# naggender2/distributed-lms-raft-llm

Hardware: AMD Instinct MI355X
Metric: tutoring tokens/sec (GPT-2-124M) + p50 query latency at 1/2/4/8 MI355X (higher is better)
Workload: dtype bf16; 1 GPU; model=gpt2 (124M), global_batch=1024, seq_len=150, prompt_len=32, decode=greedy + repetition_penalty 1.2, max_length 150 (tutoring_server.py:21-29), parallelism=dp1, hipgraph=True, device=AMD Radeon Graphics

## Files before the change

### distributed_lms_raft_llm_amd/ops/__init__.py

```python
from __future__ import annotations

import ctypes
import os
import subprocess
import threading
from pathlib import Path

import torch

_HERE = Path(__file__).resolve().parent
CSRC = _HERE / "csrc"
LIB_DIR = _HERE / "_lib"
LIB_PATH = LIB_DIR / "libdlms_hip.so"
CHECKED_LIB_PATH = LIB_DIR / "libdlms_hip_checked.so"
CHECK_UNITS = ("gemm", "attention", "decode", "encoder", "skinny", "gemm_ps", "sample")
CHECK_SITES = {1: "embed token id", 2: "position id", 3: "decode_update slot_map", 4: "decode_update token id",
               5: "decode_update sequence length", 6: "seen_set row", 7: "QKV scatter slot", 8: "QKV scatter position",
               9: "attention slot", 10: "BERT token id", 11: "seen_set token id", 12: "sampler slot_map",
               13: "sampled token id"}
SOURCES = ["api.hip", "gemm.hip", "norm.hip", "attention.hip", "decode.hip", "encoder.hip", "xgmi.hip", "skinny.hip", "gemm_ps.hip",
           "dataflow.hip", "mid.hip", "sample.hip"]
ARCH = os.environ.get("DLMS_OFFLOAD_ARCH", "gfx950")

EPI_BF16, EPI_GELU_TANH, EPI_GELU_ERF, EPI_F32, EPI_QKV, EPI_ARGMAX, EPI_PARTIAL = range(7)
# ... 1028 lines not shown

def fix_copies() -> int:
    return int(lib().dlms_fix_copies())


def fix_to_float(r: torch.Tensor) -> torch.Tensor:
    return (r.sum(0).to(torch.float64) / FIX_SCALE).to(torch.float32)


SKINNY_MLP_WIDTHS = (768, 1024, 1280, 1600)


def skinny_mlp_cg(K: int, M: int, want: int = 0) -> int:
    return int(lib().dlms_skinny_mlp_cg(K, M, want))


def skinny_mlp(x_in: torch.Tensor, gamma, beta, eps: float, w_fc_sh: torch.Tensor, b_fc, w_p_sl: torch.Tensor, b_p,
               r_out: torch.Tensor, *, parts=None, nsplit: int = 0, res_bias=None, cg: int = 0, base: bool = True):
    xfix = x_in.dtype == torch.int64
    C = fix_copies()
    xcs = 0
    if xfix:
        _req(x_in, torch.int64, "x_in", 3)
        if x_in.shape[0] != C or x_in.stride(0) % 2:
            raise ValueError(f"skinny_mlp: fixed-point x_in must be [{C}, M, d]")
        xcs = x_in.stride(0)
        x_in = x_in[0]
    else:
        _req(x_in, torch.float32, "x_in", 2)
    _req(r_out, torch.int64, "r_out", 3)
    if r_out.shape[0] != C or r_out.stride(0) % 2:
        raise ValueError(f"skinny_mlp: r_out must be [{C}, M, d]")
    rcs = r_out.stride(0)
    r_full, r_out = r_out, r_out[0]
    _req(w_fc_sh, torch.bfloat16, "w_fc_sh", 4)
    _req(w_p_sl, torch.bfloat16, "w_p_sl", 3)
    M, K = x_in.shape
    F = w_fc_sh.shape[0] * 16
    if w_fc_sh.shape[1] * 32 != K or not w_fc_sh.is_contiguous() or tuple(w_p_sl.shape) != (F // 16, K, 16) or \
            not w_p_sl.is_contiguous():
        raise ValueError("skinny_mlp: weight layouts (shuffle_weight / slice_cproj) do not match x_in")
    if M < 1 or M > 8 or K not in SKINNY_MLP_WIDTHS:
        raise ValueError(f"skinny_mlp: M <= 8 rows of width {SKINNY_MLP_WIDTHS}, got {tuple(x_in.shape)}")
    if skinny_mlp_cg(K, M, cg) == 0:
        raise ValueError(f"skinny_mlp: {M} rows of width {K} do not fit the kernel's LDS")
    if r_out.shape[0] < M or r_out.shape[1] < K or r_out.stride(1) != 1 or r_out.data_ptr() == x_in.data_ptr():
        raise ValueError("skinny_mlp: r_out too small or aliases x_in")
    if x_in.stride(1) != 1 or x_in.stride(0) % 4 or x_in.data_ptr() % 16:
        raise ValueError("skinny_mlp: x rows must be 16-byte aligned")
    for t, n, size in ((gamma, "gamma", K), (beta, "beta", K), (b_fc, "b_fc", F), (b_p, "b_p", K)):
        _req(t, torch.float32, n, 1)
        if t.numel() != size:
            raise ValueError(f"skinny_mlp: {n} size")
    if nsplit not in (0, 1, 4) or (nsplit == 4 and K > 1024):
        raise ValueError("skinny_mlp: nsplit in {0, 1, 4} (4: d <= 1024)")
    ldp, sstride = 0, 0
    if nsplit:
        _req(parts, torch.float32, "parts", 3)
        if parts.shape[0] < nsplit or parts.shape[1] < M or parts.shape[2] < K or parts.stride(2) != 1 or \
                parts.stride(1) % 4 or parts.stride(0) % 4:
            raise ValueError("skinny_mlp: parts too small / misaligned")
        ldp, sstride = parts.stride(1), parts.stride(0)
    if res_bias is not None:
        _req(res_bias, torch.float32, "res_bias", 1)
        if res_bias.numel() != K:
            raise ValueError("res_bias size")
    _check(lib().dlms_skinny_mlp(_p(x_in), x_in.stride(0), int(xfix), xcs, _p(parts) if nsplit else None, ldp,
                                 sstride, nsplit, _p(res_bias), _p(gamma), _p(beta), float(eps), _p(w_fc_sh), _p(b_fc),
                                 _p(w_p_sl), _p(b_p), _p(r_out), r_out.stride(0), rcs, M, K, F, int(cg), int(bool(base)),
                                 _stream()),
           "dlms_skinny_mlp")
    return r_full


def ln_fix(x: torch.Tensor, gamma, beta, eps: float, out: torch.Tensor):
    _req(x, torch.int64, "x", 3)
    _req(out, torch.bfloat16, "out", 2)
    if x.shape[0] != fix_copies() or x.stride(0) % 2:
        raise ValueError(f"ln_fix: x must be [{fix_copies()}, M, K]")
    xcs, x = x.stride(0), x[0]
    M, K = x.shape
    if x.stride(1) != 1 or out.stride(1) != 1 or out.shape[0] < M or out.shape[1] < K or x.stride(0) % 2 or \
            out.stride(0) % 4 or K % 4 or K > 2048 or x.data_ptr() % 16 or out.data_ptr() % 8:
        raise ValueError("ln_fix: shapes / alignment")
    for t, n in ((gamma, "gamma"), (beta, "beta")):
        _req(t, torch.float32, n, 1)
        if t.numel() != K:
            raise ValueError(f"ln_fix: {n} size")
    _check(lib().dlms_ln_fix(_p(x), x.stride(0), xcs, _p(gamma), _p(beta), float(eps), _p(out), out.stride(0), M, K,
                             _stream()), "dlms_ln_fix")
    return out


def attention_split_waves(kv_len_max: int) -> int:
    for nw in (2, 4, 8, 16):
        if kv_len_max <= 32 * nw:
            return nw
    return 16


ATTN_WS_STRIDE = 68
ATTN_SPLIT_SYNC = 2


def attention_split_geometry(pairs: int, kv_len_max: int, cus: int = 256) -> tuple[int, int]:
    nw = attention_split_waves(kv_len_max)
    if pairs <= 32 and kv_len_max > 512:
        return 8, 4
    return nw, 1


class AttnSplitWorkspace:

    def __init__(self, pairs: int, splits: int, device):
        self.pairs, self.splits = pairs, splits
        self.partials = torch.empty(pairs * splits * ATTN_WS_STRIDE, dtype=torch.float32, device=device)
        self.counters = torch.zeros(pairs, dtype=torch.int32, device=device)

    def fits(self, pairs: int, splits: int) -> bool:
        return pairs <= self.pairs and pairs * splits <= self.pairs * self.splits


def attention_split(q: torch.Tensor, k_cache: torch.Tensor, v_cache: torch.Tensor, row_slot: torch.Tensor,
                    row_kvlen: torch.Tensor, out: torch.Tensor | None = None, scale: float | None = None,
                    waves: int = 16, splits: int = 1, workspace: "AttnSplitWorkspace | None" = None,
                    sync: int | None = None):
    _req(q, torch.bfloat16, "q", 2)
    kv8 = _kv_caches(k_cache, v_cache, "attention_split")
    _req(row_slot, torch.int32, "row_slot", 1)
    _req(row_kvlen, torch.int32, "row_kvlen", 1)
    R = q.shape[0]
    S, H, T, hd = k_cache.shape
    if hd != 64 or v_cache.shape != k_cache.shape or q.shape[1] < H * 64:
        raise ValueError("attention_split: bad shapes")
    if row_slot.numel() < R or row_kvlen.numel() < R:
        raise ValueError("attention_split: index arrays too short")
    if waves not in (2, 4, 8, 16):
        raise ValueError("attention_split: waves in {2, 4, 8, 16}")
    if not 1 <= splits <= 64:
        raise ValueError("attention_split: splits in [1, 64]")
    if out is None:
        out = torch.empty(R, H * 64, dtype=torch.bfloat16, device=q.device)
    _req(out, torch.bfloat16, "out", 2)
    ws_p = cnt_p = None
    if splits > 1:
        if workspace is None:
            workspace = AttnSplitWorkspace(R * H, splits, q.device)
        if not workspace.fits(R * H, splits):
            raise ValueError("attention_split: workspace too small")
        ws_p, cnt_p = _p(workspace.partials), _p(workspace.counters)
    sc = (1.0 / 8.0) if scale is None else scale
    fn = lib().dlms_attention_split_fp8 if kv8 else lib().dlms_attention_split
    _check(fn(_p(q), q.stride(0), _p(k_cache), _p(v_cache), _p(row_slot), _p(row_kvlen), _p(out), out.stride(0), R, H, T,
              S, float(sc), int(waves), int(splits), ws_p, cnt_p, ATTN_SPLIT_SYNC if sync is None else int(sync),
              _stream()), "attention_split")
    return out


def attention_oproj_tiles(n_out: int, target_wgs: int = 16) -> int:
    G = n_out // 16
    cands = [nt for nt in (2, 3, 4, 5, 6, 8) if G % nt == 0]
    if not cands:
        raise ValueError(f"attention_oproj: N/16 = {G} has no tile count in (2,3,4,5,6,8)")
    return min(cands, key=lambda nt: (abs(G // nt - target_wgs), nt))


def attention_oproj(q: torch.Tensor, k_cache: torch.Tensor, v_cache: torch.Tensor, row_slot: torch.Tensor,
                    row_kvlen: torch.Tensor, wo_sh: torch.Tensor, parts: torch.Tensor, scale: float | None = None,
                    tiles: int | None = None) -> torch.Tensor:
    _req(q, torch.bfloat16, "q", 2)
    kv8 = _kv_caches(k_cache, v_cache, "attention_oproj")
    _req(row_slot, torch.int32, "row_slot", 1)
    _req(row_kvlen, torch.int32, "row_kvlen", 1)
    _req(wo_sh, torch.bfloat16, "wo_sh", 4)
    _req(parts, torch.float32, "parts", 3)
    M = q.shape[0]
    S, H, T, hd = k_cache.shape
    N = wo_sh.shape[0] * 16
    if not 1 <= M <= 4:
        raise ValueError("attention_oproj: 1..4 rows")
    if hd != 64 or v_cache.shape != k_cache.shape or q.shape[1] < H * 64 or wo_sh.shape[1] * 32 != H * 64:
        raise ValueError("attention_oproj: bad shapes")
    if parts.shape[0] < H or parts.shape[1] < M or parts.shape[2] < N or parts.stride(2) != 1:
        raise ValueError("attention_oproj: parts must be [>= H, >= M, >= N]")
    if row_slot.numel() < M or row_kvlen.numel() < M:
        raise ValueError("attention_oproj: index arrays too short")
    nt = attention_oproj_tiles(N) if tiles is None else tiles
    sc = (1.0 / 8.0) if scale is None else scale
    fn = lib().dlms_attention_oproj_fp8 if kv8 else lib().dlms_attention_oproj
    _check(fn(_p(q), q.stride(0), _p(k_cache), _p(v_cache), _p(row_slot), _p(row_kvlen), M, H, T, S, float(sc),
              _p(wo_sh), N, int(nt), _p(parts), parts.stride(1), parts.stride(0), _stream()),
           "attention_oproj")
    return parts


def attention_oproj_grouped(q: torch.Tensor, k_cache: torch.Tensor, v_cache: torch.Tensor, row_slot: torch.Tensor,
                            row_kvlen: torch.Tensor, wo_sh: torch.Tensor, parts: torch.Tensor, heads_per_group: int,
                            scale: float | None = None, tiles: int = 3) -> torch.Tensor:
    _req(q, torch.bfloat16, "q", 2)
    kv8 = _kv_caches(k_cache, v_cache, "attention_oproj_grouped")
    _req(row_slot, torch.int32, "row_slot", 1)
    _req(row_kvlen, torch.int32, "row_kvlen", 1)
    _req(wo_sh, torch.bfloat16, "wo_sh", 4)
    _req(parts, torch.float32, "parts", 3)
    S, H, T, hd = k_cache.shape
    N = wo_sh.shape[0] * 16
    hg = int(heads_per_group)
    if q.shape[0] != 1:
        raise ValueError("attention_oproj_grouped: one row")
    if hd != 64 or v_cache.shape != k_cache.shape or q.shape[1] < H * 64 or wo_sh.shape[1] * 32 != H * 64:
        raise ValueError("attention_oproj_grouped: bad shapes")
    if hg not in (3, 4) or H % hg or (N // 16) % tiles or tiles not in (1, 2, 3, 4):
        raise ValueError("attention_oproj_grouped: heads_per_group in {3, 4} dividing H, tiles in 1..4 dividing N/16")
    if parts.shape[0] < H // hg or parts.shape[2] < N or parts.stride(2) != 1:
        raise ValueError("attention_oproj_grouped: parts must be [>= H/hg, >= 1, >= N]")
    sc = (1.0 / 8.0) if scale is None else scale
    fn = lib().dlms_attention_oproj_grouped_fp8 if kv8 else lib().dlms_attention_oproj_grouped
    _check(fn(_p(q), _p(k_cache), _p(v_cache), _p(row_slot), _p(row_kvlen), H, hg, T, S, float(sc), _p(wo_sh), N,
              int(tiles), _p(parts), parts.stride(0), _stream()),
           "attention_oproj_grouped")
    return parts


PS_WAVES = 8


PS_LDS_BYTES = 160 * 1024


def gemm_ps_geometry(M: int, N: int, epi: int, split: int = 1, cus: int = 256, K: int = 768):
    kc = K // max(1, split)
    fits4 = 64 * (kc * 2 + 32) + 8 * 4096 <= PS_LDS_BYTES
    mt = 4 if ((epi == EPI_ARGMAX or M >= 512) and fits4) else 2
    nt = 2
    row_blocks = -(-M // (16 * mt))
    tiles = N // (16 * nt)
    need = -(-tiles // PS_WAVES)
    per_row = max(1, cus // max(1, row_blocks * split))
    col_wgs = min(need, per_row) if epi == EPI_ARGMAX else need
    return mt, nt, max(1, col_wgs)


def gemm_ps(a: torch.Tensor, w_sh: torch.Tensor, epi: int, *, bias=None, out=None, q_out=None, k_cache=None,
            v_cache=None, row_slot=None, row_pos=None, argmax_out=None, seen=None, vocab: int = 0,
            col_offset: int = 0, penalty: float = 1.0, split_k: int = 1, geometry=None):
    _req(a, torch.bfloat16, "a", 2)
    _req(w_sh, torch.bfloat16, "w_sh", 4)
    if w_sh.shape[2] != 64 or w_sh.shape[3] != 8 or not w_sh.is_contiguous():
        raise ValueError("gemm_ps: w_sh must be a contiguous shuffle_weight() tensor")
    N, K = w_sh.shape[0] * 16, w_sh.shape[1] * 32
    M = a.shape[0]
    if a.shape[1] != K or a.stride(0) % 8 or a.data_ptr() % 16:
        raise ValueError(f"gemm_ps: a {tuple(a.shape)} vs K={K} (16-byte aligned rows)")
    if split_k < 1 or K % split_k or (K // split_k) % 128:
        raise ValueError("gemm_ps: K / split_k must be a multiple of 128")
    if epi != EPI_PARTIAL and split_k != 1:
        raise ValueError("gemm_ps: split_k only with EPI_PARTIAL")
    mt, nt, col_wgs = geometry or gemm_ps_geometry(M, N, epi, split_k, K=K)
    if N % (16 * nt):
        raise ValueError("gemm_ps: N must be a multiple of 16 * nt")
    ep = GemmEpi()
    if bias is not None:
        _req(bias, torch.float32, "bias", 1)
        if bias.numel() < N:
            raise ValueError("bias too short")
        ep.bias = bias.data_ptr()
    if epi in (EPI_BF16, EPI_GELU_TANH):
        if out is None:
            out = torch.empty(M, N, dtype=torch.bfloat16, device=a.device)
        _req(out, torch.bfloat16, "out", 2)
        if out.shape[0] < M or out.shape[1] < N or out.stride(0) % 8 or out.data_ptr() % 16:
            raise ValueError("gemm_ps: out too small / misaligned")
        ep.out, ep.ldo = out.data_ptr(), out.stride(0)
    elif epi == EPI_PARTIAL:
        if out is None:
            out = torch.empty(split_k, M, N, dtype=torch.float32, device=a.device)
        _req(out, torch.float32, "out", 3)
        if out.shape[0] < split_k or out.shape[1] < M or out.shape[2] < N or out.stride(1) % 4 or \
                out.stride(0) % 4 or out.data_ptr() % 16:
            raise ValueError("gemm_ps: partial out too small / misaligned")
        ep.out, ep.ldo, ep.split_k, ep.split_stride = out.data_ptr(), out.stride(1), split_k, out.stride(0)
    elif epi == EPI_QKV:
        for t, n in ((q_out, "q_out"), (k_cache, "k_cache"), (v_cache, "v_cache")):
            _req(t, torch.bfloat16, n)
        _req(row_slot, torch.int32, "row_slot", 1)
        _req(row_pos, torch.int32, "row_pos", 1)
        if N % 3 or (N // 3) % 64:
            raise ValueError("QKV N must be 3 * d_local (64-wide heads)")
        d_local = N // 3
        if k_cache.dim() != 4 or k_cache.shape != v_cache.shape or k_cache.shape[1] * 64 != d_local or \
                k_cache.shape[3] != 64 or not k_cache.is_contiguous() or not v_cache.is_contiguous():
            raise ValueError(f"cache shape {tuple(k_cache.shape)} incompatible with d_local={d_local}")
        if q_out.shape[0] < M or q_out.shape[1] < d_local or row_slot.numel() < M or row_pos.numel() < M or \
                q_out.stride(0) % 8 or q_out.data_ptr() % 16:
            raise ValueError("qkv epilogue buffers too small / misaligned")
        ep.q_out, ep.ldq = q_out.data_ptr(), q_out.stride(0)
        ep.k_cache, ep.v_cache = k_cache.data_ptr(), v_cache.data_ptr()
        ep.row_slot, ep.row_pos = row_slot.data_ptr(), row_pos.data_ptr()
        ep.n_heads, ep.t_max, ep.d_local, ep.n_slots = k_cache.shape[1], k_cache.shape[2], d_local, k_cache.shape[0]
        out = q_out
    elif epi == EPI_ARGMAX:
        _req(argmax_out, torch.int64, "argmax_out", 2)
        _req(seen, torch.int32, "seen", 2)
        slots = PS_WAVES * col_wgs
        if argmax_out.shape[0] < M or argmax_out.shape[1] < slots or seen.shape[0] < M or \
                seen.shape[1] * 32 < vocab or col_offset % 64:
            raise ValueError("gemm_ps argmax buffers too small / misaligned shard")
        ep.argmax_out, ep.ldo, ep.seen = argmax_out.data_ptr(), argmax_out.stride(0), seen.data_ptr()
        ep.seen_words, ep.vocab, ep.col_offset, ep.penalty = seen.stride(0), vocab, col_offset, penalty
        out = argmax_out
    else:
        raise ValueError(f"gemm_ps: unsupported epilogue {epi}")
    _check(lib().dlms_gemm_ps(epi, _p(a), a.stride(0), _p(w_sh), M, N, K, split_k, mt, nt, col_wgs, ctypes.byref(ep),
                              _stream()), "dlms_gemm_ps")
    return out


def gemm_ps_key_slots(M: int, N: int, K: int = 768) -> int:
    return PS_WAVES * gemm_ps_geometry(M, N, EPI_ARGMAX, K=K)[2]
```

### distributed_lms_raft_llm_amd/ops/csrc/decode.hip

```cpp
#include "common.h"

__global__ __launch_bounds__(256) void embed_kernel(const int* __restrict__ tokens, const int* __restrict__ positions,
                                                    const bf16_t* __restrict__ wte, const bf16_t* __restrict__ wpe,
                                                    float* x, int ldx, int R, int D, int V, int P) {
    const int lane = threadIdx.x & 63;
    const int r = blockIdx.x * 4 + (threadIdx.x >> 6);
    if (r >= R) return;
    const bf16_t* a = wte + (size_t)dlms_idx(tokens[r], V, CHK_EMBED_TOKEN) * D;
    const bf16_t* b = wpe + (size_t)dlms_idx(positions[r], P, CHK_EMBED_POS) * D;
    float* o = x + (size_t)r * ldx;
    for (int c = lane; c < D / 8; c += 64) {
        float fa[8], fb[8];
        unpack8(*reinterpret_cast<const uint4*>(a + c * 8), fa);
        unpack8(*reinterpret_cast<const uint4*>(b + c * 8), fb);
        float4 lo = make_float4(fa[0] + fb[0], fa[1] + fb[1], fa[2] + fb[2], fa[3] + fb[3]);
        float4 hi = make_float4(fa[4] + fb[4], fa[5] + fb[5], fa[6] + fb[6], fa[7] + fb[7]);
        reinterpret_cast<float4*>(o + c * 8)[0] = lo;
        reinterpret_cast<float4*>(o + c * 8)[1] = hi;
    }
}

#define KEY_ROUND 16
__device__ __forceinline__ void key_round_load(const unsigned long long* __restrict__ keys, int b, int nparts,
                                               long long sb, long long sp, int lane, int p0,
                                               unsigned long long (&k)[KEY_ROUND]) {
#pragma unroll
    for (int u = 0; u < KEY_ROUND; ++u) {
        const int p = p0 + lane + 64 * u;
        k[u] = keys[(size_t)b * sb + (size_t)(p < nparts ? p : nparts - 1) * sp];
    }
}
__device__ __forceinline__ unsigned long long key_round_max(const unsigned long long (&k)[KEY_ROUND], int nparts,
                                                            int lane, int p0, unsigned long long best) {
#pragma unroll
    for (int u = 0; u < KEY_ROUND; ++u) {
        const unsigned long long v = p0 + lane + 64 * u < nparts ? k[u] : 0ull;
        best = v > best ? v : best;
    }
    return best;
}
__device__ __forceinline__ unsigned long long key_rounds_from(const unsigned long long* __restrict__ keys, int b,
                                                              int nparts, long long sb, long long sp, int lane,
                                                              int p0, unsigned long long best) {
    for (; p0 < nparts; p0 += 64 * KEY_ROUND) {
        unsigned long long k[KEY_ROUND];
        key_round_load(keys, b, nparts, sb, sp, lane, p0, k);
        best = key_round_max(k, nparts, lane, p0, best);
    }
    return best;
}
__device__ __forceinline__ unsigned long long wave_key_max(const unsigned long long* __restrict__ keys, int b,
                                                           int nparts, long long sb, long long sp, int lane) {
    return wave_max_u64(key_rounds_from(keys, b, nparts, sb, sp, lane, 0, 0ull));
}

__global__ __launch_bounds__(256) void argmax_reduce_kernel(const unsigned long long* __restrict__ keys, int nparts,
                                                            long long sb, unsigned long long* out, int B) {
    const int lane = threadIdx.x & 63;
    const int b = blockIdx.x * 4 + (threadIdx.x >> 6);
    if (b >= B) return;
    const unsigned long long best = wave_key_max(keys, b, nparts, sb, 1, lane);
    if (lane == 0) out[b] = best;
}

#define DU_MAXV4 8

__global__ __launch_bounds__(256) void decode_update_kernel(const unsigned long long* __restrict__ keys, int nparts,
                                                            long long sb, long long sp,
                                                            const int* __restrict__ slot_map, int* lens,
                                                            int* finished, int* out_tokens, int max_len,
                                                            unsigned int* seen, int seen_words, int* cur_tok,
                                                            int* cur_pos, int* cur_kvlen,
                                                            const bf16_t* __restrict__ wte,
                                                            const bf16_t* __restrict__ wpe, float* x, int ldx, int B,
                                                            int D, int eos, int t_max, int n_slots, int V,
                                                            const float* __restrict__ ln_g,
                                                            const float* __restrict__ ln_b, float eps, bf16_t* h,
                                                            int ldh) {
    const int lane = threadIdx.x & 63;
    const int i = blockIdx.x * 4 + (threadIdx.x >> 6);
    if (i >= B) return;
    const int b = slot_map ? (int)dlms_idx(slot_map[i], n_slots, CHK_UPDATE_SLOT) : i;
    const int len0 = (int)dlms_idx(lens[b], max_len + 1, CHK_UPDATE_LEN);
    const int fin = finished[b];
    unsigned long long k0[KEY_ROUND];
    key_round_load(keys, i, nparts, sb, sp, lane, 0, k0);
    __builtin_amdgcn_sched_barrier(0);
    const int live_len = fin ? 0 : (int)dlms_idx(len0, max_len, CHK_UPDATE_LEN);
    int pos = fin ? len0 - 1 : live_len;
    pos = pos < 0 ? 0 : (pos < t_max - 1 ? pos : t_max - 1);
    const int prev_tok = out_tokens[(size_t)b * max_len + (len0 > 0 ? len0 - 1 : 0)];
    const int last_tok = fin ? prev_tok : 0;
    const int nv = D >> 2;
    uint2 pe[DU_MAXV4];
#pragma unroll
    for (int j = 0; j < DU_MAXV4; ++j) {
        const int c = lane + 64 * j < nv ? lane + 64 * j : nv - 1;
        pe[j] = *reinterpret_cast<const uint2*>(wpe + (size_t)pos * D + c * 4);
    }
    const float4* gsrc = reinterpret_cast<const float4*>(h ? ln_g : x + (size_t)b * ldx);
    const float4* bsrc = reinterpret_cast<const float4*>(h ? ln_b : x + (size_t)b * ldx);
    float4 lg[DU_MAXV4], lb[DU_MAXV4];
#pragma unroll
    for (int j = 0; j < DU_MAXV4; ++j) {
        const int c = lane + 64 * j < nv ? lane + 64 * j : nv - 1;
        lg[j] = gsrc[c];
        lb[j] = bsrc[c];
    }
    const unsigned long long best = wave_max_u64(
        key_rounds_from(keys, i, nparts, sb, sp, lane, 64 * KEY_ROUND, key_round_max(k0, nparts, lane, 0, 0ull)));

    int tok;
    if (!fin) {
        tok = best ? (int)(~(unsigned int)(best & 0xffffffffull)) : eos;
        tok = (int)dlms_idx(tok, V, CHK_UPDATE_TOKEN);
    } else {
        tok = (int)dlms_idx(last_tok, V, CHK_UPDATE_TOKEN);
    }
    if (lane == 0) {
        if (!fin) {
            out_tokens[(size_t)b * max_len + live_len] = tok;
            atomicOr(seen + (size_t)b * seen_words + (tok >> 5), 1u << (tok & 31));
            lens[b] = live_len + 1;
            if (tok == eos || live_len + 1 >= max_len) finished[b] = 1;
        }
        cur_tok[b] = tok;
        cur_pos[b] = pos;
        cur_kvlen[b] = pos + 1;
    }
    const bf16_t* a = wte + (size_t)tok * D;
    float4* o = reinterpret_cast<float4*>(x + (size_t)b * ldx);
    float4 v[DU_MAXV4];
    uint2 te[DU_MAXV4];
#pragma unroll
    for (int j = 0; j < DU_MAXV4; ++j)
        te[j] = *reinterpret_cast<const uint2*>(a + (lane + 64 * j < nv ? lane + 64 * j : nv - 1) * 4);
#pragma unroll
    for (int j = 0; j < DU_MAXV4; ++j) {
        const int c = lane + 64 * j;
        v[j] = make_float4(0.f, 0.f, 0.f, 0.f);
        if (c >= nv) continue;
        const uint2 e = te[j];
        v[j] = make_float4(bf16_to_f32((bf16_t)(e.x & 0xffffu)) + bf16_to_f32((bf16_t)(pe[j].x & 0xffffu)),
                           bf16_to_f32((bf16_t)(e.x >> 16)) + bf16_to_f32((bf16_t)(pe[j].x >> 16)),
                           bf16_to_f32((bf16_t)(e.y & 0xffffu)) + bf16_to_f32((bf16_t)(pe[j].y & 0xffffu)),
                           bf16_to_f32((bf16_t)(e.y >> 16)) + bf16_to_f32((bf16_t)(pe[j].y >> 16)));
        o[c] = v[j];
    }
    if (h == nullptr) return;
    float s = 0.f;
#pragma unroll
    for (int j = 0; j < DU_MAXV4; ++j) s += (v[j].x + v[j].y) + (v[j].z + v[j].w);
    const float mean = wave_sum(s) / (float)D;
    float ss = 0.f;
#pragma unroll
    for (int j = 0; j < DU_MAXV4; ++j) {
        if (lane + 64 * j < nv) {
            const float p = v[j].x - mean, q = v[j].y - mean, r = v[j].z - mean, t = v[j].w - mean;
            ss += (p * p + q * q) + (r * r + t * t);
        }
    }
    const float rstd = rsqrtf(wave_sum(ss) / (float)D + eps);
#pragma unroll
    for (int j = 0; j < DU_MAXV4; ++j) {
        const int c = lane + 64 * j;
        if (c >= nv) continue;
        const float4 g = lg[j], be = lb[j];
        uint2 pk;
        pk.x = pack_bf16x2((v[j].x - mean) * rstd * g.x + be.x, (v[j].y - mean) * rstd * g.y + be.y);
        pk.y = pack_bf16x2((v[j].z - mean) * rstd * g.z + be.z, (v[j].w - mean) * rstd * g.w + be.w);
        reinterpret_cast<uint2*>(h + (size_t)b * ldh)[c] = pk;
    }
}

extern "C" hipError_t dlms_embed(const int* tokens, const int* positions, const void* wte, const void* wpe, float* x,
                                 int ldx, int R, int D, int V, int P, hipStream_t stream) {
    if (D % 8 != 0 || R <= 0) return hipErrorInvalidValue;
    hipLaunchKernelGGL(embed_kernel, dim3((R + 3) / 4), dim3(256), 0, stream, tokens, positions,
                       reinterpret_cast<const bf16_t*>(wte), reinterpret_cast<const bf16_t*>(wpe), x, ldx, R, D, V, P);
    return hipGetLastError();
}

extern "C" hipError_t dlms_decode_update(const unsigned long long* keys, int nparts, long long sb, long long sp,
                                         const int* slot_map, int* lens, int* finished, int* out_tokens, int max_len,
                                         unsigned int* seen, int seen_words, int* cur_tok, int* cur_pos,
                                         int* cur_kvlen, const void* wte, const void* wpe, float* x, int ldx, int B,
                                         int D, int eos, int t_max, int n_slots, int V, const float* ln_g,
                                         const float* ln_b, float eps, void* h, int ldh, hipStream_t stream) {
    if (D % 8 != 0 || D > 64 * DU_MAXV4 * 4 || B <= 0 || nparts <= 0 || (h && (!ln_g || !ln_b || ldh % 4)))
        return hipErrorInvalidValue;
    hipLaunchKernelGGL(decode_update_kernel, dim3((B + 3) / 4), dim3(256), 0, stream, keys, nparts, sb, sp, slot_map,
                       lens, finished, out_tokens, max_len, seen, seen_words, cur_tok, cur_pos, cur_kvlen,
                       reinterpret_cast<const bf16_t*>(wte), reinterpret_cast<const bf16_t*>(wpe), x, ldx, B, D, eos,
                       t_max, n_slots, V, ln_g, ln_b, eps, reinterpret_cast<bf16_t*>(h), ldh);
    return hipGetLastError();
}

extern "C" hipError_t dlms_argmax_reduce(const unsigned long long* keys, int nparts, long long sb,
                                         unsigned long long* out, int B, hipStream_t stream) {
    if (B <= 0 || nparts <= 0) return hipErrorInvalidValue;
    hipLaunchKernelGGL(argmax_reduce_kernel, dim3((B + 3) / 4), dim3(256), 0, stream, keys, nparts, sb, out, B);
    return hipGetLastError();
}

__global__ __launch_bounds__(256) void seen_set_kernel(const int* __restrict__ tokens, const int* __restrict__ rows,
                                                       int R, unsigned int* seen, int seen_words, int n_rows) {
    const int i = blockIdx.x * 256 + threadIdx.x;
    if (i >= R) return;
    const int t = tokens[i];
    if (t < 0 || (t >> 5) >= seen_words) {
        dlms_idx(t, (long long)seen_words * 32, CHK_SEEN_TOKEN);
        return;
    }
    const size_t row = dlms_idx(rows[i], n_rows, CHK_SEEN_ROW);
    atomicOr(seen + row * seen_words + (t >> 5), 1u << (t & 31));
}

extern "C" hipError_t dlms_seen_set(const int* tokens, const int* rows, int R, unsigned int* seen, int seen_words,
                                    int n_rows, hipStream_t stream) {
    if (R <= 0 || seen_words <= 0) return hipErrorInvalidValue;
    hipLaunchKernelGGL(seen_set_kernel, dim3((R + 255) / 256), dim3(256), 0, stream, tokens, rows, R, seen, seen_words,
                       n_rows);
    return hipGetLastError();
}

DLMS_CHECK_EXPORT(decode)
```

### distributed_lms_raft_llm_amd/ops/csrc/gemm_ps.hip

```cpp
#include "common.h"

enum { PS_BF16 = 0, PS_GELU_TANH = 1, PS_QKV = 4, PS_ARGMAX = 5, PS_PARTIAL = 6 };

typedef __attribute__((address_space(3))) void ps_lds_void_t;
typedef __attribute__((address_space(1))) void ps_glob_void_t;

#define PS_NW 8
#define PS_KBC 4
#define PS_PAD 32
#define PS_STAGE 4096

template <int EPI, int MT, int NT, int KBC = PS_KBC, int NB = 0>
__global__ __launch_bounds__(64 * PS_NW) void gemm_ps_kernel(const bf16_t* __restrict__ A, int lda,
                                                           const bf16_t* __restrict__ Wsh, int M, int N, int K,
                                                           int row_blocks, int split, int col_wgs, GemmEpi ep) {
    constexpr int BM = 16 * MT;
    extern __shared__ __attribute__((aligned(16))) char smem[];
    const int lane = threadIdx.x & 63;
    const int wave = threadIdx.x >> 6;
    const int g = lane >> 4, fr = lane & 15;

    const int bid = xcd_remap(blockIdx.x, gridDim.x);
    const int rb = bid % row_blocks;
    const int rest = bid / row_blocks;
    const int ks = rest % split;
    const int cw = rest / split;
    const int kc = K / split;
    const int nkb = kc >> 5;
    const int nch = nkb / KBC;
    const int m0 = rb * BM;
    const int row_bytes = kc * 2 + PS_PAD;

    {
        const int pieces = (kc * 2 + 1023) >> 10;
        const int tail_lanes = ((kc * 2) & 1023) >> 4;
        for (int p = wave; p < BM * pieces; p += PS_NW) {
            const int r = p / pieces, pc = p - r * pieces;
            const int gm = m0 + r < M ? m0 + r : M - 1;
            const bool partial = pc == pieces - 1 && tail_lanes != 0;
            if (!partial || lane < tail_lanes) {
                const char* src = reinterpret_cast<const char*>(A + (size_t)gm * lda + (size_t)ks * kc) + pc * 1024 + lane * 16;
                __builtin_amdgcn_global_load_lds((ps_glob_void_t*)src, (ps_lds_void_t*)(smem + r * row_bytes + pc * 1024),
                                                 16, 0, 0);
            }
        }
    }

    const int tiles = N / (16 * NT);
    const int slot = cw * PS_NW + wave;
    const int slots = col_wgs * PS_NW;
    const int my_tiles = slot < tiles ? (tiles - 1 - slot) / slots + 1 : 0;
    const int nsteps = my_tiles * nch;
    const int kb_base = ks * nkb;
    const int nkb_all = K >> 5;
    auto frag_ptr = [&](int step, int kb, int t) {
        const int tile = slot + (step / nch) * slots;
        const int cg = tile * NT + t;
        const int kbi = kb_base + (step % nch) * KBC + kb;
        return reinterpret_cast<const bf16x8_t*>(Wsh) + ((size_t)cg * nkb_all + kbi) * 64 + lane;
    };
    auto load = [&](bf16x8_t (&b)[KBC][NT], int step_) {
        const int step = step_ < nsteps ? step_ : nsteps - 1;
#pragma unroll
        for (int kb = 0; kb < KBC; ++kb)
#pragma unroll
            for (int t = 0; t < NT; ++t) b[kb][t] = *frag_ptr(step, kb, t);
    };

    f32x4_t acc[MT][NT];
#pragma unroll
    for (int i = 0; i < MT; ++i)
#pragma unroll
        for (int t = 0; t < NT; ++t) acc[i][t] = (f32x4_t){0.f, 0.f, 0.f, 0.f};

    unsigned long long best[EPI == PS_ARGMAX ? MT : 1][4];
#pragma unroll
    for (int i = 0; i < (EPI == PS_ARGMAX ? MT : 1); ++i)
#pragma unroll
        for (int r = 0; r < 4; ++r) best[i][r] = 0ull;

    char* stage = smem + BM * row_bytes + wave * PS_STAGE;

    unsigned int* seen_stage = reinterpret_cast<unsigned int*>(stage);
    static_assert(16 * 8 * 4 <= PS_STAGE, "the staging region holds a seen word per panel row");

    auto finish_tile = [&](int step) {
        const int tile = slot + (step / nch) * slots;
        const int col0 = tile * NT * 16;
        if constexpr (EPI == PS_ARGMAX) {
            uint4 sw[MT];
#pragma unroll
            for (int i = 0; i < MT; ++i) sw[i] = *reinterpret_cast<const uint4*>(seen_stage + 16 * i + 4 * g);
#pragma unroll
            for (int i = 0; i < MT; ++i)
#pragma unroll
                for (int r = 0; r < 4; ++r) {
                    const unsigned int bits = r == 0 ? sw[i].x : r == 1 ? sw[i].y : r == 2 ? sw[i].z : sw[i].w;
#pragma unroll
                    for (int t = 0; t < NT; ++t) {
                        const int gcol = col0 + 16 * t + fr + ep.col_offset;
                        float v = acc[i][t][r];
                        if ((bits >> (gcol & 31)) & 1u) v = v < 0.f ? v * ep.penalty : v / ep.penalty;
                        const unsigned long long key =
                            ((unsigned long long)f32_ordered(v) << 32) | (unsigned long long)(~(unsigned int)gcol);
                        if (gcol < ep.vocab && key > best[i][r]) best[i][r] = key;
                    }
                }
        } else {
            constexpr int OB = EPI == PS_PARTIAL ? 4 : 2;
            constexpr int TW = 16 * NT * OB;
            constexpr int RPP = PS_STAGE / TW;
            constexpr int PASSES = (BM + RPP - 1) / RPP;
            static_assert(RPP >= 16 && RPP % 16 == 0, "staging pass holds whole 16-row tiles");
            const int ncols = 16 * NT;
#pragma unroll
            for (int ps = 0; ps < PASSES; ++ps) {
#pragma unroll
                for (int i = 0; i < MT; ++i) {
                    if (16 * i < ps * RPP || 16 * i >= (ps + 1) * RPP) continue;
#pragma unroll
                    for (int t = 0; t < NT; ++t) {
                        const int col = col0 + 16 * t + fr;
                        const float bv = (EPI != PS_PARTIAL && ep.bias) ? ep.bias[col] : 0.f;
#pragma unroll
                        for (int r = 0; r < 4; ++r) {
                            float v = acc[i][t][r] + bv;
                            if constexpr (EPI == PS_GELU_TANH) v = gelu_tanh(v);
                            char* dst = stage + (16 * i - ps * RPP + 4 * g + r) * TW + (16 * t + fr) * OB;
                            if constexpr (OB == 4)
                                *reinterpret_cast<float*>(dst) = v;
                            else
                                *reinterpret_cast<bf16_t*>(dst) = f32_to_bf16(v);
                        }
                    }
                }
                asm volatile("s_waitcnt lgkmcnt(0)" ::: "memory");
                constexpr int CPR = TW / 16;
                for (int c = lane; c < RPP * CPR; c += 64) {
                    const int lr = c / CPR, ch = c - lr * CPR;
                    const int row = m0 + ps * RPP + lr;
                    if (row >= M || ps * RPP + lr >= BM) continue;
                    const uint4 val = *reinterpret_cast<const uint4*>(stage + lr * TW + ch * 16);
                    const int col = col0 + ch * (16 / OB);
                    if constexpr (EPI == PS_PARTIAL) {
                        *reinterpret_cast<uint4*>(reinterpret_cast<float*>(ep.out) + (size_t)ks * ep.split_stride +
                                                  (size_t)row * ep.ldo + col) = val;
                    } else if constexpr (EPI == PS_QKV) {
                        const int part = col / ep.d_local;
                        const int within = col - part * ep.d_local;
                        bf16_t* dst;
                        if (part == 0) {
                            dst = ep.q_out + (size_t)row * ep.ldq + within;
                        } else {
                            const int head = within >> 6, dim = within & 63;
                            const size_t sl = dlms_idx(ep.row_slot[row], ep.n_slots, CHK_QKV_SLOT);
                            const size_t pos = dlms_idx(ep.row_pos[row], ep.t_max, CHK_QKV_POS);
                            dst = (part == 1 ? ep.k_cache : ep.v_cache) + ((sl * ep.n_heads + head) * ep.t_max + pos) * 64 + dim;
                        }
                        *reinterpret_cast<uint4*>(dst) = val;
                    } else {
                        *reinterpret_cast<uint4*>(reinterpret_cast<bf16_t*>(ep.out) + (size_t)row * ep.ldo + col) = val;
                    }
                }
                asm volatile("s_waitcnt lgkmcnt(0)" ::: "memory");
            }
            (void)ncols;
        }
#pragma unroll
        for (int i = 0; i < MT; ++i)
#pragma unroll
            for (int t = 0; t < NT; ++t) acc[i][t] = (f32x4_t){0.f, 0.f, 0.f, 0.f};
    };

    auto seen_load = [&](int step, unsigned int& swl, unsigned int& swl2) {
        const int tile = slot + (step / nch) * slots;
        const int word = (tile * NT * 16 + ep.col_offset) >> 5;
        static_assert(NT <= 2, "a tile's columns share one seen word per row");
        static_assert(MT <= 8, "two seen words per lane cover at most 8 row tiles");
        const int srow = m0 + lane < M ? m0 + lane : M - 1;
        swl = ep.seen[(size_t)srow * ep.seen_words + word];
        if constexpr (MT > 4) {
            const int srow2 = m0 + 64 + lane < M ? m0 + 64 + lane : M - 1;
            swl2 = ep.seen[(size_t)srow2 * ep.seen_words + word];
        }
    };

    auto compute = [&](const bf16x8_t (&b)[KBC][NT], int step, unsigned int swl, unsigned int swl2) {
        const int kb0 = (step % nch) * KBC;
#pragma unroll
        for (int kb = 0; kb < KBC; ++kb) {
            bf16x8_t a[MT];
#pragma unroll
            for (int i = 0; i < MT; ++i)
                a[i] = *reinterpret_cast<const bf16x8_t*>(smem + (16 * i + fr) * row_bytes + ((kb0 + kb) * 32 + g * 8) * 2);
#pragma unroll
            for (int i = 0; i < MT; ++i)
#pragma unroll
                for (int t = 0; t < NT; ++t) acc[i][t] = __builtin_amdgcn_mfma_f32_16x16x32_bf16(a[i], b[kb][t], acc[i][t], 0, 0, 0);
        }
        if constexpr (EPI == PS_ARGMAX) {
            seen_stage[lane] = swl;
            if constexpr (MT > 4) seen_stage[64 + lane] = swl2;
        }
        if (step % nch == nch - 1) finish_tile(step);
    };

    constexpr int NBUF = NB > 0 ? NB : ((EPI == PS_ARGMAX && MT * NT >= 8) ? 2 : 4);
    static_assert(NBUF >= 2 && NBUF <= 4, "2..4 register chunks");
    bf16x8_t b[NBUF][KBC][NT];
    if (nsteps > 0) {
#pragma unroll
        for (int j = 0; j < NBUF - 1; ++j) load(b[j], j);
    }
    asm volatile("s_waitcnt vmcnt(0)" ::: "memory");
    __syncthreads();
    for (int step = 0; step < nsteps; step += NBUF) {
#pragma unroll
        for (int j = 0; j < NBUF; ++j) {
            if (j > 0 && step + j >= nsteps) break;
            unsigned int swl = 0, swl2 = 0;
            if constexpr (EPI == PS_ARGMAX) seen_load(step + j, swl, swl2);
            load(b[(j + NBUF - 1) % NBUF], step + j + NBUF - 1);
            compute(b[j], step + j, swl, swl2);
        }
    }

    if constexpr (EPI == PS_ARGMAX) {
#pragma unroll
        for (int i = 0; i < MT; ++i)
#pragma unroll
            for (int r = 0; r < 4; ++r) {
                unsigned long long k = best[i][r];
                k = row16_max_u64(k);
                const int row = m0 + 16 * i + 4 * g + r;
                if (fr == 0 && row < M) ep.argmax_out[(size_t)row * ep.ldo + slot] = k;
            }
    }
}

template <int EPI, int MT, int NT, int KBC = PS_KBC, int NB = 0>
static hipError_t launch_ps(const void* A, int lda, const void* W, int M, int N, int K, int split, int col_wgs,
                            const GemmEpi& ep, hipStream_t stream) {
    const int kc = K / split;
    const int row_blocks = (M + 16 * MT - 1) / (16 * MT);
    const size_t lds = (size_t)16 * MT * (kc * 2 + PS_PAD) + (size_t)PS_NW * PS_STAGE;
    if (lds > 160 * 1024) return hipErrorInvalidValue;
    static std::atomic<uint64_t> attr_set{0};
    if (hipError_t e = lds_opt_in(attr_set, reinterpret_cast<const void*>(&gemm_ps_kernel<EPI, MT, NT, KBC, NB>), 160 * 1024);
        e != hipSuccess)
        return e;
    hipLaunchKernelGGL((gemm_ps_kernel<EPI, MT, NT, KBC, NB>), dim3(row_blocks * split * col_wgs), dim3(64 * PS_NW), lds, stream,
                       reinterpret_cast<const bf16_t*>(A), lda, reinterpret_cast<const bf16_t*>(W), M, N, K, row_blocks,
                       split, col_wgs, ep);
    return hipGetLastError();
}

extern "C" hipError_t dlms_gemm_ps(int epi, const void* A, int lda, const void* Wsh, int M, int N, int K, int split,
                                   int mt, int nt, int col_wgs, const GemmEpi* ep, hipStream_t stream) {
    if (M <= 0 || N % (16 * nt) || split < 1 || K % split || (K / split) % (32 * PS_KBC) || col_wgs < 1)
        return hipErrorInvalidValue;
    if (epi != PS_PARTIAL && split != 1) return hipErrorInvalidValue;
    if (epi == PS_ARGMAX && mt == 4 && nt == 2 && (K / split) % (32 * 8) == 0)
        return launch_ps<PS_ARGMAX, 4, 2, 8, 2>(A, lda, Wsh, M, N, K, split, col_wgs, *ep, stream);
#define PS_GEO(E)                                                                                         \
    if (mt == 2 && nt == 1) return launch_ps<E, 2, 1>(A, lda, Wsh, M, N, K, split, col_wgs, *ep, stream); \
    if (mt == 2 && nt == 2) return launch_ps<E, 2, 2>(A, lda, Wsh, M, N, K, split, col_wgs, *ep, stream); \
    if (mt == 4 && nt == 1) return launch_ps<E, 4, 1>(A, lda, Wsh, M, N, K, split, col_wgs, *ep, stream); \
    if (mt == 4 && nt == 2) return launch_ps<E, 4, 2>(A, lda, Wsh, M, N, K, split, col_wgs, *ep, stream); \
    if (E == PS_ARGMAX && mt == 5 && nt == 2) return launch_ps<PS_ARGMAX, 5, 2>(A, lda, Wsh, M, N, K, split, col_wgs, *ep, stream); \
    return hipErrorInvalidValue;
    switch (epi) {
        case PS_BF16: PS_GEO(PS_BF16)
        case PS_GELU_TANH: PS_GEO(PS_GELU_TANH)
        case PS_QKV: PS_GEO(PS_QKV)
        case PS_ARGMAX: PS_GEO(PS_ARGMAX)
        case PS_PARTIAL: PS_GEO(PS_PARTIAL)
        default: return hipErrorInvalidValue;
    }
#undef PS_GEO
}

DLMS_CHECK_EXPORT(gemm_ps)
```

Before: 769,300 tokens/s.

## Reduce argmax keys across waves in LDS before writing per-workgroup partials

The partial-sum GEMM argmax epilogue now reduces each wave's best keys through LDS and writes one key per workgroup instead of one per wave, which shrinks the partial-key array by a factor of PS_WAVES. The downstream argmax/decode_update kernels gain a fast path that loads a single key per lane when there are at most 64 parts. Tile assignment is also reordered so leftover tiles are spread across workgroups first. In exchange the epilogue adds a block barrier and LDS traffic, and the tail tiles land on different waves.

```diff
diff --git a/distributed_lms_raft_llm_amd/ops/__init__.py b/distributed_lms_raft_llm_amd/ops/__init__.py
--- a/distributed_lms_raft_llm_amd/ops/__init__.py
+++ b/distributed_lms_raft_llm_amd/ops/__init__.py
@@ -1354,8 +1354,7 @@
     elif epi == EPI_ARGMAX:
         _req(argmax_out, torch.int64, "argmax_out", 2)
         _req(seen, torch.int32, "seen", 2)
-        slots = PS_WAVES * col_wgs
-        if argmax_out.shape[0] < M or argmax_out.shape[1] < slots or seen.shape[0] < M or \
+        if argmax_out.shape[0] < M or argmax_out.shape[1] < col_wgs or seen.shape[0] < M or \
                 seen.shape[1] * 32 < vocab or col_offset % 64:
             raise ValueError("gemm_ps argmax buffers too small / misaligned shard")
         ep.argmax_out, ep.ldo, ep.seen = argmax_out.data_ptr(), argmax_out.stride(0), seen.data_ptr()
@@ -1369,4 +1368,4 @@
 
 
 def gemm_ps_key_slots(M: int, N: int, K: int = 768) -> int:
-    return PS_WAVES * gemm_ps_geometry(M, N, EPI_ARGMAX, K=K)[2]
+    return gemm_ps_geometry(M, N, EPI_ARGMAX, K=K)[2]
diff --git a/distributed_lms_raft_llm_amd/ops/csrc/decode.hip b/distributed_lms_raft_llm_amd/ops/csrc/decode.hip
--- a/distributed_lms_raft_llm_amd/ops/csrc/decode.hip
+++ b/distributed_lms_raft_llm_amd/ops/csrc/decode.hip
@@ -49,9 +49,25 @@
     }
     return best;
 }
+#define KEY_FEW 64
+__device__ __forceinline__ void key_first_load(const unsigned long long* __restrict__ keys, int b, int nparts,
+                                               long long sb, long long sp, int lane,
+                                               unsigned long long (&k)[KEY_ROUND]) {
+    if (nparts <= KEY_FEW)
+        k[0] = keys[(size_t)b * sb + (size_t)(lane < nparts ? lane : nparts - 1) * sp];
+    else
+        key_round_load(keys, b, nparts, sb, sp, lane, 0, k);
+}
+__device__ __forceinline__ unsigned long long key_first_max(const unsigned long long (&k)[KEY_ROUND], int nparts,
+                                                            int lane) {
+    if (nparts <= KEY_FEW) return lane < nparts ? k[0] : 0ull;
+    return key_round_max(k, nparts, lane, 0, 0ull);
+}
 __device__ __forceinline__ unsigned long long wave_key_max(const unsigned long long* __restrict__ keys, int b,
                                                            int nparts, long long sb, long long sp, int lane) {
-    return wave_max_u64(key_rounds_from(keys, b, nparts, sb, sp, lane, 0, 0ull));
+    unsigned long long k0[KEY_ROUND];
+    key_first_load(keys, b, nparts, sb, sp, lane, k0);
+    return wave_max_u64(key_rounds_from(keys, b, nparts, sb, sp, lane, 64 * KEY_ROUND, key_first_max(k0, nparts, lane)));
 }
 
 __global__ __launch_bounds__(256) void argmax_reduce_kernel(const unsigned long long* __restrict__ keys, int nparts,
@@ -84,7 +100,7 @@
     const int len0 = (int)dlms_idx(lens[b], max_len + 1, CHK_UPDATE_LEN);
     const int fin = finished[b];
     unsigned long long k0[KEY_ROUND];
-    key_round_load(keys, i, nparts, sb, sp, lane, 0, k0);
+    key_first_load(keys, i, nparts, sb, sp, lane, k0);
     __builtin_amdgcn_sched_barrier(0);
     const int live_len = fin ? 0 : (int)dlms_idx(len0, max_len, CHK_UPDATE_LEN);
     int pos = fin ? len0 - 1 : live_len;
@@ -108,7 +124,7 @@
         lb[j] = bsrc[c];
     }
     const unsigned long long best = wave_max_u64(
-        key_rounds_from(keys, i, nparts, sb, sp, lane, 64 * KEY_ROUND, key_round_max(k0, nparts, lane, 0, 0ull)));
+        key_rounds_from(keys, i, nparts, sb, sp, lane, 64 * KEY_ROUND, key_first_max(k0, nparts, lane)));
 
     int tok;
     if (!fin) {
diff --git a/distributed_lms_raft_llm_amd/ops/csrc/gemm_ps.hip b/distributed_lms_raft_llm_amd/ops/csrc/gemm_ps.hip
--- a/distributed_lms_raft_llm_amd/ops/csrc/gemm_ps.hip
+++ b/distributed_lms_raft_llm_amd/ops/csrc/gemm_ps.hip
@@ -49,12 +49,19 @@
     const int tiles = N / (16 * NT);
     const int slot = cw * PS_NW + wave;
     const int slots = col_wgs * PS_NW;
-    const int my_tiles = slot < tiles ? (tiles - 1 - slot) / slots + 1 : 0;
+    const int full = tiles / slots;
+    const int left = wave * col_wgs + cw;
+    const int left_tile = full * slots + left;
+    const int my_tiles = full + (left_tile < tiles ? 1 : 0);
     const int nsteps = my_tiles * nch;
+    auto tile_at = [&](int step) {
+        const int r = step / nch;
+        return r < full ? slot + r * slots : left_tile;
+    };
     const int kb_base = ks * nkb;
     const int nkb_all = K >> 5;
     auto frag_ptr = [&](int step, int kb, int t) {
-        const int tile = slot + (step / nch) * slots;
+        const int tile = tile_at(step);
         const int cg = tile * NT + t;
         const int kbi = kb_base + (step % nch) * KBC + kb;
         return reinterpret_cast<const bf16x8_t*>(Wsh) + ((size_t)cg * nkb_all + kbi) * 64 + lane;
@@ -85,7 +92,7 @@
     static_assert(16 * 8 * 4 <= PS_STAGE, "the staging region holds a seen word per panel row");
 
     auto finish_tile = [&](int step) {
-        const int tile = slot + (step / nch) * slots;
+        const int tile = tile_at(step);
         const int col0 = tile * NT * 16;
         if constexpr (EPI == PS_ARGMAX) {
             uint4 sw[MT];
@@ -173,7 +180,7 @@
     };
 
     auto seen_load = [&](int step, unsigned int& swl, unsigned int& swl2) {
-        const int tile = slot + (step / nch) * slots;
+        const int tile = tile_at(step);
         const int word = (tile * NT * 16 + ep.col_offset) >> 5;
         static_assert(NT <= 2, "a tile's columns share one seen word per row");
         static_assert(MT <= 8, "two seen words per lane cover at most 8 row tiles");
@@ -226,15 +233,29 @@
     }
 
     if constexpr (EPI == PS_ARGMAX) {
+        constexpr int KEYS_OFF = 1024;
+        static_assert(16 * 8 * 4 <= KEYS_OFF && KEYS_OFF + BM * 8 <= PS_STAGE, "keys behind the seen words");
+        unsigned long long* wave_keys = reinterpret_cast<unsigned long long*>(stage + KEYS_OFF);
 #pragma unroll
         for (int i = 0; i < MT; ++i)
 #pragma unroll
             for (int r = 0; r < 4; ++r) {
                 unsigned long long k = best[i][r];
                 k = row16_max_u64(k);
-                const int row = m0 + 16 * i + 4 * g + r;
-                if (fr == 0 && row < M) ep.argmax_out[(size_t)row * ep.ldo + slot] = k;
+                if (fr == 0) wave_keys[16 * i + 4 * g + r] = k;
             }
+        __syncthreads();
+        const int lr = threadIdx.x;
+        if (lr < BM) {
+            unsigned long long k = 0ull;
+#pragma unroll
+            for (int w = 0; w < PS_NW; ++w) {
+                const unsigned long long kw =
+                    *reinterpret_cast<const unsigned long long*>(smem + BM * row_bytes + w * PS_STAGE + KEYS_OFF + lr * 8);
+                k = kw > k ? kw : k;
+            }
+            if (m0 + lr < M) ep.argmax_out[(size_t)(m0 + lr) * ep.ldo + cw] = k;
+        }
     }
 }
 
```

New measurement: 773,600 tokens/s, median of 3. Within noise of the previous version (+0.6%).
